# sp-uhh/audio-visual-vad

Measured on NVIDIA B200. Metric: AV-VAD frames/sec (device-timed), higher is better.
Workload: dtype bf16

## Files before the change

### audio-visual-vad_b200/csrc/lstm.cu

```cuda
#include <stdlib.h>

#include <mutex>
#include <string>

#include <vector>

#include "lstm_persist.cuh"
#include "lstm_pair.cuh"

namespace avvad {

__global__ void pack_lstm_w_kernel(const float* __restrict__ w, int H, int I, int ld, __nv_bfloat16* __restrict__ out) {
  const int64_t idx = (int64_t)blockIdx.x * blockDim.x + threadIdx.x;
  const int64_t total = (int64_t)4 * H * ld;
  if (idx >= total) return;
  const int np = (int)(idx / ld), j = (int)(idx - (int64_t)np * ld);
  const int u = np >> 2, g = np & 3;
  out[idx] = __float2bfloat16_rn(j < I ? w[(int64_t)(g * H + u) * I + j] : 0.f);
}
__global__ void pack_lstm_b_kernel(const float* __restrict__ b_ih, const float* __restrict__ b_hh, int H,
                                   float* __restrict__ out) {
  const int np = blockIdx.x * blockDim.x + threadIdx.x;
  if (np >= 4 * H) return;
  const int u = np >> 2, g = np & 3;
// ... 520 lines not shown
  static int n_chunks_pref = [] {
    const char* e = getenv("AVVAD_LSTM_CHUNKS");
    int v = e ? atoi(e) : 8;
    return v < 1 ? 1 : (v > 32 ? 32 : v);
  }();
  int n_chunks = n_chunks_pref;
  while (n_chunks > 1 && T / n_chunks < 16) --n_chunks;
  if (persistent && h->layers == 2 && n_chunks > 1) {
    int dev = 0;
    AVVAD_CUDA(cudaGetDevice(&dev));
    if (!h->side || h->side_device != dev) {
      if (h->side) cudaStreamDestroy(h->side);
      for (auto& e : h->ev_chunk) {
        if (e) cudaEventDestroy(e);
        e = nullptr;
      }
      if (h->ev_done) cudaEventDestroy(h->ev_done);
      h->ev_done = nullptr;
      AVVAD_CUDA(cudaStreamCreateWithFlags(&h->side, cudaStreamNonBlocking));
      for (auto& e : h->ev_chunk) AVVAD_CUDA(cudaEventCreateWithFlags(&e, cudaEventDisableTiming));
      AVVAD_CUDA(cudaEventCreateWithFlags(&h->ev_done, cudaEventDisableTiming));
      h->side_device = dev;
    }
    __nv_bfloat16* out0 = ws.hseq[0];
    __nv_bfloat16* out1 = ws.hseq[1];
    TapeView tv0{}, tv1{};
    if (tape) {
      tv0 = tape_layer(tape, 0, H, B, T);
      tv1 = tape_layer(tape, 1, H, B, T);
      out0 = tv0.hseq;
      out1 = tv1.hseq;
    }
    const int64_t Bp = (B + 127) / 128 * 128;
    int rc = tc::launch_tma_gemm_xt(layer_in, ld_in, h->w_ih[0], ld_in, B, T, T, H4, (int)ld_in, h->bias[0], ws.xproj, st);
    if (rc) return rc;
    const int free_sms = lstm_num_sms() - 2 * (4 * H / 128);
    for (int c = 0; c < n_chunks; ++c) {
      const int t0 = (int)(T * c / n_chunks), t1 = (int)(T * (c + 1) / n_chunks);
      bool done = false;
      rc = run_recurrence_persistent(h, 0, ws.xproj, out0, lengths, B, T, ws.counters, st, &done, tv0.gates, tv0.c, t0, t1,
                                     ws.c);
      if (rc) return rc;
      if (!done) {
        set_error("lstm: persistent recurrence unavailable");
        return AVVAD_ERR_STATE;
      }
      AVVAD_CUDA(cudaEventRecord(h->ev_chunk[c], st));
      AVVAD_CUDA(cudaStreamWaitEvent(h->side, h->ev_chunk[c], 0));
      rc = tc::launch_tma_gemm_xt(out0 + (int64_t)t0 * H, H, h->w_ih[1], H, B, t1 - t0, T, H4, H, h->bias[1],
                                  ws.xproj1 + (int64_t)t0 * H4 * Bp, h->side, free_sms > 16 ? free_sms : 0);
      if (rc) return rc;
      rc = run_recurrence_persistent(h, 1, ws.xproj1, out1, lengths, B, T, ws.counters + kCounterBytes / 4, h->side, &done,
                                     tv1.gates, tv1.c, t0, t1, ws.c1);
      if (rc) return rc;
    }
    AVVAD_CUDA(cudaEventRecord(h->ev_done, h->side));
    AVVAD_CUDA(cudaStreamWaitEvent(st, h->ev_done, 0));
    layer_out = out1;
  } else {
  for (int l = 0; l < h->layers; ++l) {
    layer_out = ws.hseq[l & 1];
    TapeView tv{};
    if (tape) {
      tv = tape_layer(tape, l, H, B, T);
      layer_out = tv.hseq;
    }
    int rc = persistent ? tc::launch_tma_gemm_xt(layer_in, ld_in, h->w_ih[l], ld_in, B, T, T, H4, (int)ld_in, h->bias[l],
                                                 ws.xproj, st)
                        : avvad_gemm_bf16(layer_in, ld_in, h->w_ih[l], ld_in, h->bias[l], ws.xproj, H4, 0, 0, rows, H4,
                                          ld_in, st);
    if (rc) return rc;
// ... 89 lines not shown
```

### audio-visual-vad_b200/csrc/lstm_pair.cuh

```cuda
#pragma once
#include "lstm_persist.cuh"

namespace avvad {
namespace tc {

__host__ __device__ constexpr int kPairThreadsOf(int epi_warps) { return 64 + 32 * epi_warps; }
__host__ __device__ constexpr int kPairStagesOf(int np) { return np == 128 ? 6 : 9; }
constexpr int kPairTraceSlots = 12;

struct PairGeom {
  int B, T, H, KB;
  int n_pairs;
  const float4* xT;
  int Bp;
  __nv_bfloat16* hseq;
  const int32_t* lengths;
  unsigned int* counters;
  __nv_bfloat16* gates_out;
  float* c_out;
  int t0, t1;
  float* c_state;
  unsigned long long* trace;
  int variant;
};
// ... 105 lines not shown
  const uint32_t tmem_acc = *tmem_slot;
  const uint32_t bar0_leader = mapa_u32(bar0, 0);
  auto LBAR = [&](int i) { return bar0_leader + 8u * (uint32_t)i; };

  if (warp == 0) {
    uint32_t it = 0;
    for (int t = (g.t0 > 1 ? g.t0 : 1); t < g.t1; ++t) {
      const unsigned int target = (unsigned int)(t - g.t0);
      bool ok = false;
      int kb = 0;
      uint32_t spins = 0;
      while (kb < g.KB) {
        if (!ok) {
          if (kPerKb == 2) {
            if (lane >= g.n_pairs) {
              ok = true;
            } else {
              unsigned int fv;
              asm volatile("ld.relaxed.gpu.global.u32 %0, [%1];" : "=r"(fv) : "l"(flags + lane) : "memory");
              ok = fv >= target;
            }
          } else {
            if (2 * lane >= g.n_pairs) {
              ok = true;
            } else {
              unsigned long long fv;
              asm volatile("ld.relaxed.gpu.global.u64 %0, [%1];" : "=l"(fv) : "l"(flags + 2 * lane) : "memory");
              ok = ((unsigned int)fv >= target) && ((unsigned int)(fv >> 32) >= target);
            }
          }
          if (++spins > (1u << 26)) __trap();
        }
        const unsigned int m = __ballot_sync(0xffffffffu, ok);
        if (lane == 0 && ((m >> (2 * kb)) & 3u) == 3u) {
          if (kTrace && kb == 0) trace[t * kPairTraceSlots + 0] = globaltimer_ns();
          if (g.variant & 2) asm volatile("fence.acq_rel.gpu;" ::: "memory");
          if (g.variant & 4) fence_proxy_async_global();
        }
        while (kb < g.KB && ((m >> (2 * kb)) & 3u) == 3u) {
          if (lane == 0) {
            const int s = it % S;
            mbar_wait(BAR(S + s), ((it / S) & 1u) ^ 1u);
            if (rank == 0) mbar_arrive_expect_tx(BAR(s), 32768u);
            tma_load_3d_2sm(sA + s * 16384u, &maps.h, kb * 64, t - 1, (int)rank * 128, LBAR(s));
            if (kTrace && kb == 0) trace[t * kPairTraceSlots + 1] = globaltimer_ns();
          }
          ++kb;
          ++it;
        }
      }
      if (kTrace && lane == 0) trace[t * kPairTraceSlots + 2] = globaltimer_ns();
    }
  } else if (warp == 1) {
    if (rank == 0) {
      constexpr uint32_t idesc = make_idesc_pair(NP);
      uint32_t it = 0;
      const int tb = g.t0 > 1 ? g.t0 : 1;
      for (int t = tb; t < g.t1; ++t) {
        const uint32_t k = (uint32_t)(t - tb), a = k & 1u;
        if (k >= 2) mbar_wait(BAR(kBarTE + a), ((k >> 1) - 1u) & 1u);
        tc_fence_after();
        const uint32_t d = tmem_acc + a * (uint32_t)NP;
        for (int kb = 0; kb < g.KB; ++kb, ++it) {
          const int s = it % S;
          mbar_wait(BAR(s), (it / S) & 1u);
          tc_fence_after();
          if (elect_one_sync()) {
            if (kTrace && kb == 0) trace[t * kPairTraceSlots + 3] = globaltimer_ns();
            const uint32_t a_lo = desc_lo(sA + s * 16384u);
            const uint32_t b_lo = desc_lo(sW + kb * kWTile);
// ... 87 lines not shown
            const float gg = tanh_hw(__uint_as_float(v[o + 2]) + x[u].z);
            const float go = sigmoid_hw(__uint_as_float(v[o + 3]) + x[u].w);
            c[u] = gf * c[u] + gi_ * gg;
            hv[j] = go * tanh_hw(c[u]);
            gp.v[2 * j] = pack_bf16x2(gi_, gf);
            gp.v[2 * j + 1] = pack_bf16x2(gg, go);
          }
          hp[4 * gi + 2 * k] = live ? pack_bf16x2(hv[0], hv[1]) : 0u;
          hp[4 * gi + 2 * k + 1] = live ? pack_bf16x2(hv[2], hv[3]) : 0u;
          if (gsave) st_global_256(gsave + 32 * gi + 16 * k, gp);
        }
      }
      if (row_ok) {
        if (kU == 16) {
          u32x8 o;
#pragma unroll
          for (int e = 0; e < 8; ++e) o.v[e] = hp[e & (kU / 2 - 1)];
          st_global_256(hrow + (int64_t)t * g.H, o);
        } else {
          *reinterpret_cast<uint4*>(hrow + (int64_t)t * g.H) = make_uint4(hp[0], hp[1], hp[2], hp[3]);
        }
        if (g.c_out) {
          float* cp = g.c_out + ((int64_t)b * g.T + t) * g.H + unit0;
#pragma unroll
          for (int k = 0; k < kU / 8; ++k) {
            u32x8 o;
#pragma unroll
            for (int e = 0; e < 8; ++e) o.v[e] = __float_as_uint(c[8 * k + e]);
            st_global_256(cp + 8 * k, o);
          }
        }
      }
      if (tr) trace[t * kPairTraceSlots + 7] = globaltimer_ns();
      asm volatile("bar.sync 1, %0;" ::"n"(32 * kEW) : "memory");
      if (warp == 2 && lane == 0) {
        if (kTrace) trace[t * kPairTraceSlots + 9] = globaltimer_ns();
        asm volatile("st.release.gpu.global.u32 [%0], %1;" ::"l"(flags + pair), "r"((unsigned int)(t + 1 - g.t0))
                     : "memory");
        if (kTrace) trace[t * kPairTraceSlots + 10] = globaltimer_ns();
      }
    }
    if (row_ok && g.c_state) {
      float4* cs = reinterpret_cast<float4*>(g.c_state + (int64_t)b * g.H + unit0);
#pragma unroll
      for (int u = 0; u < kU / 4; ++u) cs[u] = make_float4(c[4 * u], c[4 * u + 1], c[4 * u + 2], c[4 * u + 3]);
    }
  }

  tc_fence_before();
  __syncthreads();
  cluster_sync_all();
  if (warp == 1) {
    __syncwarp();
    tmem_dealloc2(tmem_acc, 2 * NP);
  }
}

}
}
```

### audio-visual-vad_b200/csrc/lstm_persist.cuh

```cuda
#pragma once
#include "gemm_tma.cuh"

namespace avvad {
namespace tc {

constexpr int kLstmThreads = 320;
constexpr int kLstmStages = 6;
constexpr int kLstmMaxSlices = 64;

struct LstmGeom {
  int B, T, H, KB;
  int n_slices;
  const float4* xT;
  int Bp;
  __nv_bfloat16* hseq;
  const int32_t* lengths;
  unsigned int* counters;
  __nv_bfloat16* gates_out;
  float* c_out;
  int t0, t1;
  float* c_state;
  int cluster;
  int variant;
};
// ... 118 lines not shown
              if (++spins > (1u << 26)) __trap();
            }
            if (elect_one_sync()) {
              asm volatile("fence.acq_rel.gpu;" ::: "memory");
              fence_proxy_async_global();
              tma_load_3d_mc(sA + s * 16384u, &maps.h, kb * 64, t - 1, ms * 128, BAR(s), cmask);
            }
            __syncwarp();
          }
        }
      }
    } else {
    const int f0 = 2 * lane, f1 = 2 * lane + 1;
    const unsigned long long* fpair = reinterpret_cast<const unsigned long long*>(flags + f0);
    for (int t = (g.t0 > 1 ? g.t0 : 1); t < g.t1; ++t) {
      const unsigned int target = (unsigned int)(t - g.t0);
      bool ok = false;
      int kb = 0;
      uint32_t spins = 0;
      while (kb < g.KB) {
        if (!ok) {
          if (f0 >= g.n_slices) {
            ok = true;
          } else {
            unsigned long long fv;
            asm volatile("ld.relaxed.gpu.global.u64 %0, [%1];" : "=l"(fv) : "l"(fpair) : "memory");
            ok = ((unsigned int)fv >= target) && (f1 >= g.n_slices || (unsigned int)(fv >> 32) >= target);
          }
          if (++spins > (1u << 26)) __trap();
          if (!ok && (g.variant & 2)) __nanosleep(20);
        }
        const unsigned int m = __ballot_sync(0xffffffffu, ok);
        if (lane == 0 && kb < g.KB && ((m >> (2 * kb)) & 3u) == 3u) {
          if (g.variant & 32) asm volatile("fence.acq_rel.gpu;" ::: "memory");
          if (g.variant & 64) fence_proxy_async_global();
        }
        while (kb < g.KB && ((m >> (2 * kb)) & 3u) == 3u) {
          if (lane == 0) {
            const int s = it % kLstmStages;
            mbar_wait(BAR(kLstmStages + s), ((it / kLstmStages) & 1u) ^ 1u);
            mbar_arrive_expect_tx(BAR(s), 16384u);
            tma_load_3d(sA + s * 16384u, &maps.h, kb * 64, t - 1, ms * 128, BAR(s));
          }
          ++kb;
          ++it;
        }
      }
    }
    }
  } else if (warp == 1) {
    constexpr uint32_t idesc = make_idesc(64);
    mbar_wait(BAR(kBarW), 0);
    tc_fence_after();
    uint32_t it = 0;
    const int tb = g.t0 > 1 ? g.t0 : 1;
    for (int t = tb; t < g.t1; ++t) {
      const uint32_t k = (uint32_t)(t - tb), acc = k & 1u;
      if (k >= 2) mbar_wait(BAR(kBarTE + acc), ((k >> 1) - 1u) & 1u);
      tc_fence_after();
      const uint32_t d = tmem_acc + acc * 64u;
      for (int kb = 0; kb < g.KB; ++kb, ++it) {
        const int s = it % kLstmStages;
        mbar_wait(BAR(s), (it / kLstmStages) & 1u);
        tc_fence_after();
        if (elect_one_sync()) {
          const uint32_t a_lo = desc_lo(sA + s * 16384u);
          const uint32_t b_lo = desc_lo(sW + kb * 8192u);
          umma_f16_lo(d, a_lo, b_lo, idesc, kb != 0);
// ... 127 lines not shown
```

### audio-visual-vad_b200/csrc/stem_s2d.cuh

```cuda
#pragma once
#include "gemm_tc.cuh"

namespace avvad {
namespace tc {

constexpr int kS2Builders = 256;
constexpr int kS2BuilderWarps = kS2Builders / 32;
constexpr int kS2EpiWarps = 8;
constexpr int kS2EpiThreads = kS2EpiWarps * 32;
constexpr int kS2ChPerWarp = 64 / (kS2EpiWarps / 4);
constexpr int kS2Passes = kS2ChPerWarp / 16;
constexpr int kS2Items = (67 * 37 + kS2Builders - 1) / kS2Builders;
constexpr int kS2Threads = kS2Builders + 32 + kS2EpiThreads;
constexpr int kS2FramesPerBatch = 2;
constexpr int kS2RowsPerFrame = 37;
constexpr int kS2Pitch = 160;
constexpr int kS2PlaneRows = 83;
constexpr uint32_t kS2PlaneBytes = kS2PlaneRows * kS2Pitch;
constexpr int kS2EdgeRows = 132;
constexpr uint32_t kS2EdgeChunkBytes = kS2EdgeRows * 16;
constexpr uint32_t kS2EdgePlaneBytes = 2 * kS2EdgeChunkBytes;
constexpr uint32_t kS2BufBytes = 2 * kS2PlaneBytes + 2 * kS2EdgePlaneBytes;
constexpr uint32_t kS2WStepBytes = 256 * 32;
constexpr uint32_t kS2WBytes = 8 * kS2WStepBytes;
constexpr uint32_t kS2OnesBytes = 128 * 32;
constexpr int kS2RingRows = 32;
constexpr uint32_t kS2RingRowBytes = 16 * 128;
constexpr uint32_t kS2RingBytes = kS2RingRows * kS2RingRowBytes;
constexpr uint32_t kS2EdgeHpBytes = 80 * 128;
constexpr uint32_t kS2OffW = 2 * kS2BufBytes;
constexpr uint32_t kS2OffOnes = kS2OffW + kS2WBytes;
constexpr uint32_t kS2OffRing = kS2OffOnes + kS2OnesBytes;
constexpr uint32_t kS2OffEdgeHp = kS2OffRing + kS2RingBytes;
constexpr uint32_t kS2OffLut = kS2OffEdgeHp + kS2EdgeHpBytes;
constexpr uint32_t kS2OffBias = kS2OffLut + 512;
constexpr uint32_t kS2OffBar = kS2OffBias + 256;
constexpr uint32_t kS2StageBytes = 288 * 16;
constexpr uint32_t kS2OffStage = kS2OffBar + 128;
constexpr uint32_t kS2Smem = 1024 + kS2OffStage + 2 * kS2StageBytes;
static_assert(kS2Smem <= 227 * 1024, "stem kernel: shared memory");

struct StemS2Params {
  const float* frames;
  const uint8_t* src;
  const int32_t* n_src;
  const int32_t* n_out;
  int f_max, t_max, num, den;
  float mean, denom;
  int standardise;
  int64_t n_frames;
  int64_t first;
  const __nv_bfloat16* w1b;
  int64_t src_bytes;
  const float* bias;
  __nv_bfloat16* out;
  double* stats;
};

__device__ __forceinline__ uint32_t desc_lo_ns(uint32_t saddr, uint32_t lbo_bytes) {
  return ((saddr & 0x3FFFFu) >> 4) | ((lbo_bytes >> 4) << 16);
}
__device__ __forceinline__ uint32_t desc_hi_ns(uint32_t sbo_bytes) { return (sbo_bytes >> 4) | (1u << 14); }

__device__ __forceinline__ void umma_f16_ns(uint32_t tmem_d, uint32_t a_lo, uint32_t a_hi, uint32_t b_lo, uint32_t b_hi,
                                            uint32_t idesc, uint32_t accum) {
  asm volatile(
      "{\n\t.reg .pred p;\n\t.reg .b64 da, db;\n\t"
      "mov.b64 da, {%1, %2};\n\t"
      "mov.b64 db, {%3, %4};\n\t"
      "setp.ne.b32 p, %6, 0;\n\t"
      "tcgen05.mma.cta_group::1.kind::f16 [%0], da, db, %5, p;\n\t}"
      ::"r"(tmem_d), "r"(a_lo), "r"(a_hi), "r"(b_lo), "r"(b_hi), "r"(idesc), "r"(accum)
      : "memory");
}

__device__ __forceinline__ int s2_src_index(int k, int n_src, int num, int den) {
  long long v = ((long long)den * (2LL * k + 1) - 1) / (2LL * num);
  return v < n_src - 1 ? (int)v : n_src - 1;
}

__device__ __forceinline__ void named_bar_sync(int id, int nthreads) {
  asm volatile("bar.sync %0, %1;" ::"r"(id), "r"(nthreads) : "memory");
}

__device__ __forceinline__ uint32_t bf16x2_max(uint32_t a, uint32_t b) {
  uint32_t r;
  asm("max.bf16x2 %0, %1, %2;" : "=r"(r) : "r"(a), "r"(b));
  return r;
}

template <int MODE, bool STATS = false>
__global__ void __launch_bounds__(kS2Threads, 1) stem_s2d_kernel(const StemS2Params p) {
  extern __shared__ uint8_t smem_raw[];
  const uint32_t raw = smem_u32(smem_raw);
  const uint32_t base = (raw + 1023u) & ~1023u;
  uint8_t* smem = smem_raw + (base - raw);
  float* bias_s = reinterpret_cast<float*>(smem + kS2OffBias);
  unsigned short* lut = reinterpret_cast<unsigned short*>(smem + kS2OffLut);
  const uint32_t bar0 = base + kS2OffBar;
  auto BAR = [&](int i) { return bar0 + 8u * (uint32_t)i; };
  volatile uint32_t* tmem_slot = reinterpret_cast<volatile uint32_t*>(smem + kS2OffBar + 96);

  const int tid = threadIdx.x;
  const int warp = tid >> 5, lane = tid & 31;
  const int64_t n_batches = (p.n_frames + kS2FramesPerBatch - 1) / kS2FramesPerBatch;

  for (uint32_t i = tid; i < (2 * kS2BufBytes) / 16; i += kS2Threads)
    reinterpret_cast<uint4*>(smem)[i] = make_uint4(0u, 0u, 0u, 0u);
  for (int idx = tid; idx < 7 * 256 * 16; idx += kS2Threads) {
    const int e = idx & 15, n = (idx >> 4) & 255, fr = idx >> 12;
    const int s = n >> 6, ch = n & 63;
    const int fs = e - 2 * s;
    __nv_bfloat16 v = __float2bfloat16_rn(0.f);
    if (fs >= 0 && fs < 7) v = p.w1b[ch * 64 + fr * 7 + fs];
    const uint32_t off = kS2OffW + (uint32_t)fr * kS2WStepBytes + (uint32_t)(n >> 3) * 256u + (uint32_t)(e >> 3) * 128u +
                         (uint32_t)(n & 7) * 16u + (uint32_t)(e & 7) * 2u;
    *reinterpret_cast<__nv_bfloat16*>(smem + off) = v;
  }
  for (int idx = tid; idx < 256 * 16; idx += kS2Threads) {
    const int e = idx & 15, n = idx >> 4;
    const float bv = p.bias ? p.bias[n & 63] : 0.f;
    const __nv_bfloat16 hi = __float2bfloat16_rn(bv);
    __nv_bfloat16 v = __float2bfloat16_rn(0.f);
    if (e == 0) v = hi;
    if (e == 1) v = __float2bfloat16_rn(bv - __bfloat162float(hi));
    const uint32_t off = kS2OffW + 7u * kS2WStepBytes + (uint32_t)(n >> 3) * 256u + (uint32_t)(e >> 3) * 128u +
                         (uint32_t)(n & 7) * 16u + (uint32_t)(e & 7) * 2u;
    *reinterpret_cast<__nv_bfloat16*>(smem + off) = v;
  }
  for (uint32_t i = tid; i < kS2OnesBytes / 4; i += kS2Threads)
    reinterpret_cast<uint32_t*>(smem + kS2OffOnes)[i] = 0x3F803F80u;
  if (tid < 64) bias_s[tid] = p.bias ? p.bias[tid] : 0.f;
  if (MODE == 1 && tid < 256) {
    float v = (float)tid;
    if (p.standardise) v = (v - p.mean) / p.denom;
    const __nv_bfloat16 h = __float2bfloat16_rn(v);
    lut[tid] = *reinterpret_cast<const unsigned short*>(&h);
  }
  if (tid == 0) {
    for (int i = 0; i < 2; ++i) {
      mbar_init(BAR(0 + i), kS2Builders);
      mbar_init(BAR(2 + i), 1);
      mbar_init(BAR(4 + i), 1);
      mbar_init(BAR(6 + i), kS2EpiWarps);
    }
    fence_barrier_init();
  }
  if (warp == kS2BuilderWarps) {
    tmem_alloc(smem_u32(const_cast<uint32_t*>(tmem_slot)), 512);
    tmem_relinquish();
  }
  fence_proxy_async();
  tc_fence_before();
  __syncthreads();
  tc_fence_after();
  const uint32_t tmem_acc = *tmem_slot;

  if (warp < kS2BuilderWarps) {
    uint32_t px[MODE == 0 ? kS2Items : 1];
    uint4 ck0 = make_uint4(0u, 0u, 0u, 0u), ck1 = ck0;
    bool live_next = false;
    uint32_t mis_next = 0;
    auto load_chunk = [&](const uint8_t* ptr) -> uint4 {
      if (ptr >= p.src && ptr + 16 <= p.src + p.src_bytes) return __ldg(reinterpret_cast<const uint4*>(ptr));
      uint32_t w[4] = {0u, 0u, 0u, 0u};
      for (int i = 0; i < 16; ++i)
        if (ptr + i >= p.src && ptr + i < p.src + p.src_bytes) w[i >> 2] |= (uint32_t)__ldg(ptr + i) << (8 * (i & 3));
      return make_uint4(w[0], w[1], w[2], w[3]);
    };
    auto fetch = [&](int64_t n) {
      if (MODE == 1) live_next = false;
      if (n >= p.n_frames) return;
      if (MODE == 0) {
        const float* f32 = p.frames + n * (67 * 67);
#pragma unroll
        for (int j = 0; j < kS2Items; ++j) {
          const int item = tid + j * kS2Builders;
          const int r = item / 37, q = item - r * 37;
// ... 95 lines not shown
      for (int t = -1; t < n_main; ++t, ++g) {
        const uint32_t acc = g & 1u;
        mbar_wait(BAR(6 + acc), ((g >> 1) & 1u) ^ 1u);
        tc_fence_after();
        if (elect_one_sync()) {
          const uint32_t d = tmem_acc + acc * 256u;
          umma_f16_ns(d, desc_lo_ns(base + kS2OffOnes, 128u), b_hi, desc_lo_ns(base + kS2OffW + 7u * kS2WStepBytes, 128u),
                      b_hi, idesc, 0);
#pragma unroll
          for (int fr = 0; fr < 7; ++fr) {
            const int a = fr >> 1, b = fr & 1;
            uint32_t a_lo, a_hi;
            if (t < 0) {
              a_lo = desc_lo_ns(bufa + 2 * kS2PlaneBytes + (uint32_t)b * kS2EdgePlaneBytes + (uint32_t)a * 16u,
                                kS2EdgeChunkBytes);
              a_hi = a_hi_edge;
            } else {
              a_lo = desc_lo_ns(bufa + (uint32_t)b * kS2PlaneBytes + (uint32_t)(16 * t + a) * kS2Pitch, 16u);
              a_hi = a_hi_main;
            }
            const uint32_t b_lo = desc_lo_ns(base + kS2OffW + (uint32_t)fr * kS2WStepBytes, 128u);
            umma_f16_ns(d, a_lo, a_hi, b_lo, b_hi, idesc, 1);
          }
          umma_commit(BAR(4 + acc));
          if (t == n_main - 1) umma_commit(BAR(2 + buf));
        }
        __syncwarp();
      }
    }
  } else {
    const int ew = warp - (kS2BuilderWarps + 1);
    const int q = warp & 3;
    const int half = ew >> 2;
    const int etid = tid - (kS2Builders + 32);
    const int L = q * 32 + lane;
    uint8_t* ring = smem + kS2OffRing;
    uint8_t* edge_hp = smem + kS2OffEdgeHp;
    uint32_t g = 0;
    if (STATS) {
      float sa[kS2ChPerWarp], sq[kS2ChPerWarp];
#pragma unroll
      for (int c = 0; c < kS2ChPerWarp; ++c) sa[c] = sq[c] = 0.f;
      for (int64_t bi = blockIdx.x; bi < n_batches; bi += gridDim.x) {
        const int nf = (int)((p.n_frames - bi * kS2FramesPerBatch) < kS2FramesPerBatch
                                 ? (p.n_frames - bi * kS2FramesPerBatch)
                                 : kS2FramesPerBatch);
        const int n_rows = nf * kS2RowsPerFrame;
        const int n_main = (n_rows + 15) / 16;
        for (int t = -1; t < n_main; ++t, ++g) {
          const uint32_t acc = g & 1u;
          mbar_wait(BAR(4 + acc), (g >> 1) & 1u);
          tc_fence_after();
          const uint32_t t_row = tmem_acc + acc * 256u + ((uint32_t)(q * 32) << 16);
          const int yy = (t < 0) ? L : 16 * t + (L >> 3);
          const int y = yy % kS2RowsPerFrame;
          const bool live = (yy < n_rows) && (y < 34) && (t >= 0 || L < 80);
          const int s_first = (t < 0) ? 2 : 0;
#pragma unroll 1
          for (int pass = 0; pass < kS2Passes; ++pass) {
            const int ch0 = half * kS2ChPerWarp + pass * 16;
#pragma unroll
            for (int sft = 0; sft < 4; ++sft) {
              uint32_t v[16];
              tmem_ld16(t_row + (uint32_t)sft * 64u + ch0, v);
              tmem_ld_wait();
              if (live && sft >= s_first) {
#pragma unroll
                for (int c = 0; c < 16; ++c) {
                  const float x = __uint_as_float(v[c]);
                  if (kS2Passes == 1 || pass == 0) {
                    sa[c] += x;
                    sq[c] = fmaf(x, x, sq[c]);
                  } else {
                    sa[(16 + c) % kS2ChPerWarp] += x;
                    sq[(16 + c) % kS2ChPerWarp] = fmaf(x, x, sq[(16 + c) % kS2ChPerWarp]);
                  }
                }
              }
            }
          }
          tc_fence_before();
          __syncwarp();
          if (lane == 0) mbar_arrive(BAR(6 + acc));
        }
      }
#pragma unroll
      for (int c = 0; c < kS2ChPerWarp; ++c) {
        float a = sa[c], b = sq[c];
#pragma unroll
        for (int o = 16; o > 0; o >>= 1) {
          a += __shfl_xor_sync(0xffffffffu, a, o);
          b += __shfl_xor_sync(0xffffffffu, b, o);
        }
        if (lane == 0) {
          atomicAdd(p.stats + half * kS2ChPerWarp + c, (double)a);
          atomicAdd(p.stats + 64 + half * kS2ChPerWarp + c, (double)b);
        }
      }
    } else
    for (int64_t bi = blockIdx.x; bi < n_batches; bi += gridDim.x) {
      const int nf = (int)((p.n_frames - bi * kS2FramesPerBatch) < kS2FramesPerBatch
                               ? (p.n_frames - bi * kS2FramesPerBatch)
                               : kS2FramesPerBatch);
      const int n_rows = nf * kS2RowsPerFrame;
      const int n_main = (n_rows + 15) / 16;
      for (int t = -1; t < n_main; ++t, ++g) {
        const uint32_t acc = g & 1u;
        mbar_wait(BAR(4 + acc), (g >> 1) & 1u);
        tc_fence_after();
        const uint32_t t_row = tmem_acc + acc * 256u + ((uint32_t)(q * 32) << 16);
        if (t < 0) {
#pragma unroll 1
          for (int pass = 0; pass < kS2Passes; ++pass) {
            const int ch0 = half * kS2ChPerWarp + pass * 16;
            uint32_t v1[16], v2[16], v3[16];
            tmem_ld16(t_row + 64u + ch0, v1);
            tmem_ld16(t_row + 128u + ch0, v2);
            tmem_ld16(t_row + 192u + ch0, v3);
            tmem_ld_wait();
            if (L < 80) {
              uint32_t o[8];
#pragma unroll
              for (int c = 0; c < 8; ++c) {
                const float x0 = fmaxf(fmaxf(__uint_as_float(v1[2 * c]), __uint_as_float(v2[2 * c])), __uint_as_float(v3[2 * c]));
                const float x1 = fmaxf(fmaxf(__uint_as_float(v1[2 * c + 1]), __uint_as_float(v2[2 * c + 1])),
                                       __uint_as_float(v3[2 * c + 1]));
                o[c] = pack_relu_bf16x2(x0, x1);
              }
              uint8_t* rowp = edge_hp + L * 128;
              const int k0 = ch0 >> 3;
              *reinterpret_cast<uint4*>(rowp + (((k0) ^ (L & 7)) << 4)) = make_uint4(o[0], o[1], o[2], o[3]);
              *reinterpret_cast<uint4*>(rowp + (((k0 + 1) ^ (L & 7)) << 4)) = make_uint4(o[4], o[5], o[6], o[7]);
            }
          }
          tc_fence_before();
          __syncwarp();
          if (lane == 0) mbar_arrive(BAR(6 + acc));
          named_bar_sync(1, kS2EpiThreads);
          continue;
        }
        const int yy = 16 * t + (L >> 3);
        const int i = L & 7;
        uint8_t* rrow = ring + (uint32_t)(yy & (kS2RingRows - 1)) * kS2RingRowBytes;
#pragma unroll 1
        for (int pass = 0; pass < kS2Passes; ++pass) {
          const int ch0 = half * kS2ChPerWarp + pass * 16;
          uint32_t v0[16], v1[16], v2[16], v3[16];
          tmem_ld16(t_row + ch0, v0);
          tmem_ld16(t_row + 64u + ch0, v1);
          tmem_ld16(t_row + 128u + ch0, v2);
          tmem_ld16(t_row + 192u + ch0, v3);
          tmem_ld_wait();
          uint32_t oa[8], ob[8];
#pragma unroll
          for (int c = 0; c < 16; c += 2) {
            float pa[2], pb[2];
#pragma unroll
            for (int h = 0; h < 2; ++h) {
              const float s0 = __uint_as_float(v0[c + h]), s1 = __uint_as_float(v1[c + h]);
              const float s2 = __uint_as_float(v2[c + h]), s3 = __uint_as_float(v3[c + h]);
              float left = __shfl_up_sync(0xffffffffu, s3, 1);
              left = (i == 0) ? s0 : left;
              pa[h] = fmaxf(fmaxf(left, s0), s1);
              pb[h] = fmaxf(fmaxf(s1, s2), s3);
            }
            oa[c >> 1] = pack_relu_bf16x2(pa[0], pa[1]);
            ob[c >> 1] = pack_relu_bf16x2(pb[0], pb[1]);
          }
          if (yy < n_rows) {
            const int k0 = ch0 >> 3;
            uint8_t* pxa = rrow + (2 * i) * 128;
            uint8_t* pxb = pxa + 128;
            *reinterpret_cast<uint4*>(pxa + (((k0) ^ i) << 4)) = make_uint4(oa[0], oa[1], oa[2], oa[3]);
            *reinterpret_cast<uint4*>(pxa + (((k0 + 1) ^ i) << 4)) = make_uint4(oa[4], oa[5], oa[6], oa[7]);
            *reinterpret_cast<uint4*>(pxb + (((k0) ^ i) << 4)) = make_uint4(ob[0], ob[1], ob[2], ob[3]);
            *reinterpret_cast<uint4*>(pxb + (((k0 + 1) ^ i) << 4)) = make_uint4(ob[4], ob[5], ob[6], ob[7]);
          }
        }
        tc_fence_before();
        __syncwarp();
        if (lane == 0) mbar_arrive(BAR(6 + acc));
        named_bar_sync(1, kS2EpiThreads);

        {
          const int ch = etid & 7, rr = (etid >> 3) & 7, pg = etid >> 6;
          int ys = 16 * t + 2 * rr;
          int fi = (ys >= kS2RowsPerFrame) ? 1 : 0;
          int y = ys - fi * kS2RowsPerFrame;
          if ((y & 1) == 0) {
            ++ys; ++y;
            if (y == kS2RowsPerFrame) { y = 0; ++fi; }
          }
          if ((y & 1) && y <= 33 && ys < n_rows && fi < nf) {
            const int ph = y >> 1;
            const uint8_t* r0 = ring + (uint32_t)(ys & (kS2RingRows - 1)) * kS2RingRowBytes;
            const uint8_t* r1 = ring + (uint32_t)((ys - 1) & (kS2RingRows - 1)) * kS2RingRowBytes;
            const uint8_t* r2 = ring + (uint32_t)((ys - 2) & (kS2RingRows - 1)) * kS2RingRowBytes;
            const bool top = (y >= 2);
            __nv_bfloat16* orow = p.out + ((bi * kS2FramesPerBatch + fi) * 17 + ph) * (17 * 64) + ch * 8;
#pragma unroll
            for (int pw = pg; pw < 17; pw += kS2EpiThreads / 64) {
              uint4 a, b, c;
              if (pw < 16) {
                const uint32_t off = (uint32_t)pw * 128u + (uint32_t)((ch ^ (pw >> 1)) << 4);
                a = *reinterpret_cast<const uint4*>(r0 + off);
                b = *reinterpret_cast<const uint4*>(r1 + off);
                c = top ? *reinterpret_cast<const uint4*>(r2 + off) : b;
              } else {
                a = *reinterpret_cast<const uint4*>(edge_hp + ys * 128 + ((ch ^ (ys & 7)) << 4));
                b = *reinterpret_cast<const uint4*>(edge_hp + (ys - 1) * 128 + ((ch ^ ((ys - 1) & 7)) << 4));
                c = top ? *reinterpret_cast<const uint4*>(edge_hp + (ys - 2) * 128 + ((ch ^ ((ys - 2) & 7)) << 4)) : b;
              }
              uint4 m;
              m.x = bf16x2_max(bf16x2_max(a.x, b.x), c.x);
              m.y = bf16x2_max(bf16x2_max(a.y, b.y), c.y);
              m.z = bf16x2_max(bf16x2_max(a.z, b.z), c.z);
              m.w = bf16x2_max(bf16x2_max(a.w, b.w), c.w);
              *reinterpret_cast<uint4*>(orow + pw * 64) = m;
            }
          }
        }
        named_bar_sync(1, kS2EpiThreads);
      }
    }
  }

  tc_fence_before();
  __syncthreads();
  if (warp == kS2BuilderWarps) {
    __syncwarp();
    tmem_dealloc(tmem_acc, 512);
  }
}

}
}
```

Before: 2.138 million.

## Chunk layer-0 input projection per chunk and make memory-ordering fences default

Measured after the change: 2.136 million, median of 6. Within noise of the previous version (-0.1%).

```diff
diff --git a/audio-visual-vad_b200/csrc/lstm.cu b/audio-visual-vad_b200/csrc/lstm.cu
--- a/audio-visual-vad_b200/csrc/lstm.cu
+++ b/audio-visual-vad_b200/csrc/lstm.cu
@@ -576,11 +576,13 @@
       out1 = tv1.hseq;
     }
     const int64_t Bp = (B + 127) / 128 * 128;
-    int rc = tc::launch_tma_gemm_xt(layer_in, ld_in, h->w_ih[0], ld_in, B, T, T, H4, (int)ld_in, h->bias[0], ws.xproj, st);
-    if (rc) return rc;
     const int free_sms = lstm_num_sms() - 2 * (4 * H / 128);
     for (int c = 0; c < n_chunks; ++c) {
       const int t0 = (int)(T * c / n_chunks), t1 = (int)(T * (c + 1) / n_chunks);
+      int rc = tc::launch_tma_gemm_xt(layer_in + (int64_t)t0 * ld_in, ld_in, h->w_ih[0], ld_in, B, t1 - t0, T, H4, (int)ld_in,
+                                      h->bias[0], ws.xproj + (int64_t)t0 * H4 * Bp, st,
+                                      (c > 0 && free_sms > 16) ? free_sms : 0);
+      if (rc) return rc;
       bool done = false;
       rc = run_recurrence_persistent(h, 0, ws.xproj, out0, lengths, B, T, ws.counters, st, &done, tv0.gates, tv0.c, t0, t1,
                                      ws.c);
diff --git a/audio-visual-vad_b200/csrc/lstm_pair.cuh b/audio-visual-vad_b200/csrc/lstm_pair.cuh
--- a/audio-visual-vad_b200/csrc/lstm_pair.cuh
+++ b/audio-visual-vad_b200/csrc/lstm_pair.cuh
@@ -161,10 +161,22 @@
           if (++spins > (1u << 26)) __trap();
         }
         const unsigned int m = __ballot_sync(0xffffffffu, ok);
-        if (lane == 0 && ((m >> (2 * kb)) & 3u) == 3u) {
-          if (kTrace && kb == 0) trace[t * kPairTraceSlots + 0] = globaltimer_ns();
-          if (g.variant & 2) asm volatile("fence.acq_rel.gpu;" ::: "memory");
-          if (g.variant & 4) fence_proxy_async_global();
+        if (((m >> (2 * kb)) & 3u) == 3u) {
+          if (kTrace && kb == 0 && lane == 0) trace[t * kPairTraceSlots + 0] = globaltimer_ns();
+          int kb_end = kb + 1;
+          while (kb_end < g.KB && ((m >> (2 * kb_end)) & 3u) == 3u) ++kb_end;
+          const int lkb = lane >> 1;
+          if (!(g.variant & 2) && lkb >= kb && lkb < kb_end && kPerKb * lane < 2 * g.n_pairs) {
+            if (kPerKb == 2) {
+              unsigned int fv;
+              asm volatile("ld.acquire.gpu.global.u32 %0, [%1];" : "=r"(fv) : "l"(flags + lane) : "memory");
+            } else {
+              unsigned long long fv;
+              asm volatile("ld.acquire.gpu.global.u64 %0, [%1];" : "=l"(fv) : "l"(flags + 2 * lane) : "memory");
+            }
+          }
+          __syncwarp();
+          if (lane == 0 && !(g.variant & 4)) fence_proxy_async_global();
         }
         while (kb < g.KB && ((m >> (2 * kb)) & 3u) == 3u) {
           if (lane == 0) {
@@ -318,6 +330,8 @@
         }
       }
       if (tr) trace[t * kPairTraceSlots + 7] = globaltimer_ns();
+      if (!(g.variant & 8)) fence_proxy_async_global();
+      if (tr) trace[t * kPairTraceSlots + 8] = globaltimer_ns();
       asm volatile("bar.sync 1, %0;" ::"n"(32 * kEW) : "memory");
       if (warp == 2 && lane == 0) {
         if (kTrace) trace[t * kPairTraceSlots + 9] = globaltimer_ns();
diff --git a/audio-visual-vad_b200/csrc/lstm_persist.cuh b/audio-visual-vad_b200/csrc/lstm_persist.cuh
--- a/audio-visual-vad_b200/csrc/lstm_persist.cuh
+++ b/audio-visual-vad_b200/csrc/lstm_persist.cuh
@@ -174,8 +174,8 @@
         }
         const unsigned int m = __ballot_sync(0xffffffffu, ok);
         if (lane == 0 && kb < g.KB && ((m >> (2 * kb)) & 3u) == 3u) {
-          if (g.variant & 32) asm volatile("fence.acq_rel.gpu;" ::: "memory");
-          if (g.variant & 64) fence_proxy_async_global();
+          if (!(g.variant & 32)) asm volatile("fence.acq_rel.gpu;" ::: "memory");
+          if (!(g.variant & 64)) fence_proxy_async_global();
         }
         while (kb < g.KB && ((m >> (2 * kb)) & 3u) == 3u) {
           if (lane == 0) {
```

## Replace shared-ring epilogue with register pooling and per-warp carry barriers

Applied to the files above, without the earlier changes.

Result: no change. 2.126 million before, 2.135 million after (median of 6 runs) (+0.4%).

```diff
diff --git a/audio-visual-vad_b200/csrc/stem_s2d.cuh b/audio-visual-vad_b200/csrc/stem_s2d.cuh
--- a/audio-visual-vad_b200/csrc/stem_s2d.cuh
+++ b/audio-visual-vad_b200/csrc/stem_s2d.cuh
@@ -12,10 +12,12 @@
 constexpr int kS2Passes = kS2ChPerWarp / 16;
 constexpr int kS2Items = (67 * 37 + kS2Builders - 1) / kS2Builders;
 constexpr int kS2Threads = kS2Builders + 32 + kS2EpiThreads;
-constexpr int kS2FramesPerBatch = 2;
+constexpr int kS2FramesPerBatch = 3;
 constexpr int kS2RowsPerFrame = 37;
+constexpr int kS2BatchRows = kS2FramesPerBatch * kS2RowsPerFrame;
+constexpr int kS2MainTiles = (kS2BatchRows + 15) / 16;
 constexpr int kS2Pitch = 160;
-constexpr int kS2PlaneRows = 83;
+constexpr int kS2PlaneRows = 16 * kS2MainTiles + 3;
 constexpr uint32_t kS2PlaneBytes = kS2PlaneRows * kS2Pitch;
 constexpr int kS2EdgeRows = 132;
 constexpr uint32_t kS2EdgeChunkBytes = kS2EdgeRows * 16;
@@ -24,19 +26,24 @@
 constexpr uint32_t kS2WStepBytes = 256 * 32;
 constexpr uint32_t kS2WBytes = 8 * kS2WStepBytes;
 constexpr uint32_t kS2OnesBytes = 128 * 32;
-constexpr int kS2RingRows = 32;
-constexpr uint32_t kS2RingRowBytes = 16 * 128;
-constexpr uint32_t kS2RingBytes = kS2RingRows * kS2RingRowBytes;
-constexpr uint32_t kS2EdgeHpBytes = 80 * 128;
+constexpr int kS2CarrySlots = 4;
+constexpr uint32_t kS2CarrySlotBytes = 2 * 32 * 16;
+constexpr uint32_t kS2CarryBytes = kS2EpiWarps * kS2CarrySlots * kS2CarrySlotBytes;
+constexpr uint32_t kS2EdgeHpBytes = 16 * ((kS2BatchRows + 15) / 16) * 128;
+constexpr int kS2NumBars = 8 + kS2EpiWarps * kS2CarrySlots;
 constexpr uint32_t kS2OffW = 2 * kS2BufBytes;
 constexpr uint32_t kS2OffOnes = kS2OffW + kS2WBytes;
-constexpr uint32_t kS2OffRing = kS2OffOnes + kS2OnesBytes;
-constexpr uint32_t kS2OffEdgeHp = kS2OffRing + kS2RingBytes;
+constexpr uint32_t kS2OffCarry = kS2OffOnes + kS2OnesBytes;
+constexpr uint32_t kS2OffEdgeHp = kS2OffCarry + kS2CarryBytes;
 constexpr uint32_t kS2OffLut = kS2OffEdgeHp + kS2EdgeHpBytes;
 constexpr uint32_t kS2OffBias = kS2OffLut + 512;
 constexpr uint32_t kS2OffBar = kS2OffBias + 256;
+constexpr uint32_t kS2OffTmemSlot = kS2OffBar + 8 * kS2NumBars;
 constexpr uint32_t kS2StageBytes = 288 * 16;
-constexpr uint32_t kS2OffStage = kS2OffBar + 128;
+constexpr uint32_t kS2OffStage = kS2OffBar + 512;
+static_assert(kS2OffTmemSlot + 4 <= kS2OffStage, "stem kernel: barrier area");
+static_assert(kS2BatchRows <= 128, "stem kernel: the edge tile holds one stream row per accumulator row");
+static_assert(kS2EpiWarps == 8 && kS2Passes == 2, "stem kernel: the epilogue is written for 8 warps x 32 channels");
 constexpr uint32_t kS2Smem = 1024 + kS2OffStage + 2 * kS2StageBytes;
 static_assert(kS2Smem <= 227 * 1024, "stem kernel: shared memory");
 
@@ -88,6 +95,20 @@
   asm("max.bf16x2 %0, %1, %2;" : "=r"(r) : "r"(a), "r"(b));
   return r;
 }
+__device__ __forceinline__ uint4 bf16x2_max4(uint4 a, uint4 b) {
+  return make_uint4(bf16x2_max(a.x, b.x), bf16x2_max(a.y, b.y), bf16x2_max(a.z, b.z), bf16x2_max(a.w, b.w));
+}
+
+__device__ __forceinline__ void tmem_ld_16x256b_x2(uint32_t taddr, uint32_t (&v)[8]) {
+  asm volatile("tcgen05.ld.sync.aligned.16x256b.x2.b32 {%0, %1, %2, %3, %4, %5, %6, %7}, [%8];"
+               : "=r"(v[0]), "=r"(v[1]), "=r"(v[2]), "=r"(v[3]), "=r"(v[4]), "=r"(v[5]), "=r"(v[6]), "=r"(v[7])
+               : "r"(taddr)
+               : "memory");
+}
+
+__host__ __device__ constexpr int s2_col_channel(int c) {
+  return (c & 32) + 8 * ((c >> 1) & 3) + 2 * ((c >> 3) & 3) + (c & 1);
+}
 
 template <int MODE, bool STATS = false>
 __global__ void __launch_bounds__(kS2Threads, 1) stem_s2d_kernel(const StemS2Params p) {
@@ -99,7 +120,7 @@
   unsigned short* lut = reinterpret_cast<unsigned short*>(smem + kS2OffLut);
   const uint32_t bar0 = base + kS2OffBar;
   auto BAR = [&](int i) { return bar0 + 8u * (uint32_t)i; };
-  volatile uint32_t* tmem_slot = reinterpret_cast<volatile uint32_t*>(smem + kS2OffBar + 96);
+  volatile uint32_t* tmem_slot = reinterpret_cast<volatile uint32_t*>(smem + kS2OffTmemSlot);
 
   const int tid = threadIdx.x;
   const int warp = tid >> 5, lane = tid & 31;
@@ -109,7 +130,7 @@
     reinterpret_cast<uint4*>(smem)[i] = make_uint4(0u, 0u, 0u, 0u);
   for (int idx = tid; idx < 7 * 256 * 16; idx += kS2Threads) {
     const int e = idx & 15, n = (idx >> 4) & 255, fr = idx >> 12;
-    const int s = n >> 6, ch = n & 63;
+    const int s = n >> 6, ch = s2_col_channel(n & 63);
     const int fs = e - 2 * s;
     __nv_bfloat16 v = __float2bfloat16_rn(0.f);
     if (fs >= 0 && fs < 7) v = p.w1b[ch * 64 + fr * 7 + fs];
@@ -119,7 +140,7 @@
   }
   for (int idx = tid; idx < 256 * 16; idx += kS2Threads) {
     const int e = idx & 15, n = idx >> 4;
-    const float bv = p.bias ? p.bias[n & 63] : 0.f;
+    const float bv = p.bias ? p.bias[s2_col_channel(n & 63)] : 0.f;
     const __nv_bfloat16 hi = __float2bfloat16_rn(bv);
     __nv_bfloat16 v = __float2bfloat16_rn(0.f);
     if (e == 0) v = hi;
@@ -144,6 +165,8 @@
       mbar_init(BAR(4 + i), 1);
       mbar_init(BAR(6 + i), kS2EpiWarps);
     }
+    for (int i = 0; i < kS2EpiWarps * kS2CarrySlots; ++i) mbar_init(BAR(8 + i), 1);
+
     fence_barrier_init();
   }
   if (warp == kS2BuilderWarps) {
@@ -305,9 +328,7 @@
     const int ew = warp - (kS2BuilderWarps + 1);
     const int q = warp & 3;
     const int half = ew >> 2;
-    const int etid = tid - (kS2Builders + 32);
     const int L = q * 32 + lane;
-    uint8_t* ring = smem + kS2OffRing;
     uint8_t* edge_hp = smem + kS2OffEdgeHp;
     uint32_t g = 0;
     if (STATS) {
@@ -327,7 +348,7 @@
           const uint32_t t_row = tmem_acc + acc * 256u + ((uint32_t)(q * 32) << 16);
           const int yy = (t < 0) ? L : 16 * t + (L >> 3);
           const int y = yy % kS2RowsPerFrame;
-          const bool live = (yy < n_rows) && (y < 34) && (t >= 0 || L < 80);
+          const bool live = (yy < n_rows) && (y < 34);
           const int s_first = (t < 0) ? 2 : 0;
 #pragma unroll 1
           for (int pass = 0; pass < kS2Passes; ++pass) {
@@ -366,134 +387,157 @@
           b += __shfl_xor_sync(0xffffffffu, b, o);
         }
         if (lane == 0) {
-          atomicAdd(p.stats + half * kS2ChPerWarp + c, (double)a);
-          atomicAdd(p.stats + 64 + half * kS2ChPerWarp + c, (double)b);
-        }
-      }
-    } else
-    for (int64_t bi = blockIdx.x; bi < n_batches; bi += gridDim.x) {
-      const int nf = (int)((p.n_frames - bi * kS2FramesPerBatch) < kS2FramesPerBatch
-                               ? (p.n_frames - bi * kS2FramesPerBatch)
-                               : kS2FramesPerBatch);
-      const int n_rows = nf * kS2RowsPerFrame;
-      const int n_main = (n_rows + 15) / 16;
-      for (int t = -1; t < n_main; ++t, ++g) {
-        const uint32_t acc = g & 1u;
-        mbar_wait(BAR(4 + acc), (g >> 1) & 1u);
-        tc_fence_after();
-        const uint32_t t_row = tmem_acc + acc * 256u + ((uint32_t)(q * 32) << 16);
-        if (t < 0) {
-#pragma unroll 1
-          for (int pass = 0; pass < kS2Passes; ++pass) {
-            const int ch0 = half * kS2ChPerWarp + pass * 16;
-            uint32_t v1[16], v2[16], v3[16];
-            tmem_ld16(t_row + 64u + ch0, v1);
-            tmem_ld16(t_row + 128u + ch0, v2);
-            tmem_ld16(t_row + 192u + ch0, v3);
-            tmem_ld_wait();
-            if (L < 80) {
-              uint32_t o[8];
-#pragma unroll
-              for (int c = 0; c < 8; ++c) {
-                const float x0 = fmaxf(fmaxf(__uint_as_float(v1[2 * c]), __uint_as_float(v2[2 * c])), __uint_as_float(v3[2 * c]));
-                const float x1 = fmaxf(fmaxf(__uint_as_float(v1[2 * c + 1]), __uint_as_float(v2[2 * c + 1])),
-                                       __uint_as_float(v3[2 * c + 1]));
-                o[c] = pack_relu_bf16x2(x0, x1);
+          const int ch = s2_col_channel(half * kS2ChPerWarp + c);
+          atomicAdd(p.stats + ch, (double)a);
+          atomicAdd(p.stats + 64 + ch, (double)b);
+        }
+      }
+    } else {
+      const int gi = lane >> 2, u = lane & 3;
+      const int qp = (q + 3) & 3;
+      const int chunk = half * 4 + u;
+      const int bar_out = 8 + (half * 4 + q) * kS2CarrySlots, bar_in = 8 + (half * 4 + qp) * kS2CarrySlots;
+      uint8_t* carry_out = smem + kS2OffCarry + (uint32_t)(half * 4 + q) * kS2CarrySlots * kS2CarrySlotBytes;
+      const uint8_t* carry_in = smem + kS2OffCarry + (uint32_t)(half * 4 + qp) * kS2CarrySlots * kS2CarrySlotBytes;
+      for (int64_t bi = blockIdx.x; bi < n_batches; bi += gridDim.x) {
+        const int nf = (int)((p.n_frames - bi * kS2FramesPerBatch) < kS2FramesPerBatch
+                                 ? (p.n_frames - bi * kS2FramesPerBatch)
+                                 : kS2FramesPerBatch);
+        const int n_rows = nf * kS2RowsPerFrame;
+        const int n_main = (n_rows + 15) / 16;
+        __nv_bfloat16* out_b = p.out + bi * kS2FramesPerBatch * (17 * 17 * 64) + chunk * 8;
+        auto out_px = [&](int r, int pw) {
+          const int fi = r / kS2RowsPerFrame, y = r - fi * kS2RowsPerFrame;
+          return reinterpret_cast<uint4*>(out_b + ((fi * 17 + (y >> 1)) * 17 + pw) * 64);
+        };
+        auto trigger = [&](int r) {
+          const int y = r % kS2RowsPerFrame;
+          return (y & 1) && y <= 33 && r < n_rows;
+        };
+        auto has_top = [&](int r) { return r % kS2RowsPerFrame >= 2; };
+        for (int t = -1; t < n_main; ++t, ++g) {
+          const uint32_t acc = g & 1u, slot = g % kS2CarrySlots;
+          mbar_wait(BAR(4 + acc), (g >> 1) & 1u);
+          tc_fence_after();
+          const uint32_t t_q = tmem_acc + acc * 256u + ((uint32_t)(q * 32) << 16) + (uint32_t)(half * 32);
+          if (t < 0) {
+            uint32_t e[4][4];
+#pragma unroll
+            for (int pass = 0; pass < 2; ++pass) {
+              uint32_t v[2][3][8];
+#pragma unroll
+              for (int h = 0; h < 2; ++h)
+#pragma unroll
+                for (int s = 1; s < 4; ++s)
+                  tmem_ld_16x256b_x2(t_q + ((uint32_t)(16 * h) << 16) + (uint32_t)(64 * s + 16 * pass), v[h][s - 1]);
+              tmem_ld_wait();
+#pragma unroll
+              for (int h = 0; h < 2; ++h)
+#pragma unroll
+                for (int m = 0; m < 2; ++m)
+#pragma unroll
+                  for (int k = 0; k < 2; ++k) {
+                    const int x = 4 * k + 2 * m;
+                    float o[2];
+#pragma unroll
+                    for (int c = 0; c < 2; ++c)
+                      o[c] = fmaxf(fmaxf(__uint_as_float(v[h][0][x + c]), __uint_as_float(v[h][1][x + c])),
+                                   __uint_as_float(v[h][2][x + c]));
+                    e[2 * h + m][2 * pass + k] = pack_relu_bf16x2(o[0], o[1]);
+                  }
+            }
+            tc_fence_before();
+            __syncwarp();
+            if (lane == 0) mbar_arrive(BAR(6 + acc));
+#pragma unroll
+            for (int j = 0; j < 4; ++j) {
+              const int r = 32 * q + 8 * j + gi;
+              if (r < n_rows)
+                *reinterpret_cast<uint4*>(edge_hp + r * 128 + ((chunk ^ gi) << 4)) =
+                    make_uint4(e[j][0], e[j][1], e[j][2], e[j][3]);
+            }
+            __syncwarp();
+            if (lane == 0) mbar_arrive(BAR(bar_out + slot));
+            if (q > 0) mbar_wait(BAR(bar_in + slot), (g / kS2CarrySlots) & 1u);
+#pragma unroll
+            for (int j = 0; j < 4; ++j) {
+              const int r = 32 * q + 8 * j + gi;
+              if (trigger(r)) {
+                auto row = [&](int rr) {
+                  return *reinterpret_cast<const uint4*>(edge_hp + rr * 128 + ((chunk ^ (rr & 7)) << 4));
+                };
+                uint4 mx = bf16x2_max4(make_uint4(e[j][0], e[j][1], e[j][2], e[j][3]), row(r - 1));
+                if (has_top(r)) mx = bf16x2_max4(mx, row(r - 2));
+                *out_px(r, 16) = mx;
               }
-              uint8_t* rowp = edge_hp + L * 128;
-              const int k0 = ch0 >> 3;
-              *reinterpret_cast<uint4*>(rowp + (((k0) ^ (L & 7)) << 4)) = make_uint4(o[0], o[1], o[2], o[3]);
-              *reinterpret_cast<uint4*>(rowp + (((k0 + 1) ^ (L & 7)) << 4)) = make_uint4(o[4], o[5], o[6], o[7]);
             }
+            continue;
+          }
+          uint32_t hp[4][2][4];
+#pragma unroll
+          for (int pass = 0; pass < 2; ++pass)
+#pragma unroll
+            for (int h = 0; h < 2; ++h) {
+              uint32_t v[4][8];
+#pragma unroll
+              for (int s = 0; s < 4; ++s)
+                tmem_ld_16x256b_x2(t_q + ((uint32_t)(16 * h) << 16) + (uint32_t)(64 * s + 16 * pass), v[s]);
+              tmem_ld_wait();
+#pragma unroll
+              for (int m = 0; m < 2; ++m)
+#pragma unroll
+                for (int k = 0; k < 2; ++k) {
+                  const int x = 4 * k + 2 * m;
+                  auto f = [&](int s, int c) { return __uint_as_float(v[s][x + c]); };
+                  const uint32_t left = __shfl_up_sync(0xffffffffu, pack_relu_bf16x2(f(3, 0), f(3, 1)), 4);
+                  const uint32_t p01 = pack_relu_bf16x2(fmaxf(f(0, 0), f(1, 0)), fmaxf(f(0, 1), f(1, 1)));
+                  hp[2 * h + m][0][2 * pass + k] = (gi == 0) ? p01 : bf16x2_max(left, p01);
+                  hp[2 * h + m][1][2 * pass + k] = pack_relu_bf16x2(fmaxf(fmaxf(f(1, 0), f(2, 0)), f(3, 0)),
+                                                                    fmaxf(fmaxf(f(1, 1), f(2, 1)), f(3, 1)));
+                }
           }
           tc_fence_before();
           __syncwarp();
           if (lane == 0) mbar_arrive(BAR(6 + acc));
-          named_bar_sync(1, kS2EpiThreads);
-          continue;
-        }
-        const int yy = 16 * t + (L >> 3);
-        const int i = L & 7;
-        uint8_t* rrow = ring + (uint32_t)(yy & (kS2RingRows - 1)) * kS2RingRowBytes;
-#pragma unroll 1
-        for (int pass = 0; pass < kS2Passes; ++pass) {
-          const int ch0 = half * kS2ChPerWarp + pass * 16;
-          uint32_t v0[16], v1[16], v2[16], v3[16];
-          tmem_ld16(t_row + ch0, v0);
-          tmem_ld16(t_row + 64u + ch0, v1);
-          tmem_ld16(t_row + 128u + ch0, v2);
-          tmem_ld16(t_row + 192u + ch0, v3);
-          tmem_ld_wait();
-          uint32_t oa[8], ob[8];
-#pragma unroll
-          for (int c = 0; c < 16; c += 2) {
-            float pa[2], pb[2];
-#pragma unroll
-            for (int h = 0; h < 2; ++h) {
-              const float s0 = __uint_as_float(v0[c + h]), s1 = __uint_as_float(v1[c + h]);
-              const float s2 = __uint_as_float(v2[c + h]), s3 = __uint_as_float(v3[c + h]);
-              float left = __shfl_up_sync(0xffffffffu, s3, 1);
-              left = (i == 0) ? s0 : left;
-              pa[h] = fmaxf(fmaxf(left, s0), s1);
-              pb[h] = fmaxf(fmaxf(s1, s2), s3);
+          auto row4 = [&](int j, int c) { return make_uint4(hp[j][c][0], hp[j][c][1], hp[j][c][2], hp[j][c][3]); };
+
+          const int r_first = 16 * t + 4 * q;
+          {
+            const int y0 = (r_first + 4) % kS2RowsPerFrame;
+            const bool two = (y0 & 1) && y0 >= 3;
+            uint4* cp = reinterpret_cast<uint4*>(carry_out + slot * kS2CarrySlotBytes);
+#pragma unroll
+            for (int c = 0; c < 2; ++c) cp[32 * c + lane] = two ? bf16x2_max4(row4(3, c), row4(2, c)) : row4(3, c);
+          }
+          __syncwarp();
+          if (lane == 0) mbar_arrive(BAR(bar_out + slot));
+
+          uint4 cin[2] = {};
+          if (trigger(r_first) || (trigger(r_first + 1) && has_top(r_first + 1))) {
+            const uint32_t gp = q ? g : g - 1;
+            mbar_wait(BAR(bar_in + gp % kS2CarrySlots), (gp / kS2CarrySlots) & 1u);
+            const uint4* cp = reinterpret_cast<const uint4*>(carry_in + (gp % kS2CarrySlots) * kS2CarrySlotBytes);
+#pragma unroll
+            for (int c = 0; c < 2; ++c) cin[c] = cp[32 * c + lane];
+          }
+#pragma unroll
+          for (int j = 0; j < 4; ++j) {
+            const int r = r_first + j;
+            if (!trigger(r)) continue;
+            const bool top = has_top(r);
+#pragma unroll
+            for (int c = 0; c < 2; ++c) {
+              uint4 mx;
+              if (j == 0) {
+                mx = bf16x2_max4(row4(0, c), cin[c]);
+              } else {
+                mx = bf16x2_max4(row4(j, c), row4(j - 1, c));
+                if (top) mx = bf16x2_max4(mx, j == 1 ? cin[c] : row4(j >= 2 ? j - 2 : 0, c));
+              }
+              *out_px(r, 2 * gi + c) = mx;
             }
-            oa[c >> 1] = pack_relu_bf16x2(pa[0], pa[1]);
-            ob[c >> 1] = pack_relu_bf16x2(pb[0], pb[1]);
-          }
-          if (yy < n_rows) {
-            const int k0 = ch0 >> 3;
-            uint8_t* pxa = rrow + (2 * i) * 128;
-            uint8_t* pxb = pxa + 128;
-            *reinterpret_cast<uint4*>(pxa + (((k0) ^ i) << 4)) = make_uint4(oa[0], oa[1], oa[2], oa[3]);
-            *reinterpret_cast<uint4*>(pxa + (((k0 + 1) ^ i) << 4)) = make_uint4(oa[4], oa[5], oa[6], oa[7]);
-            *reinterpret_cast<uint4*>(pxb + (((k0) ^ i) << 4)) = make_uint4(ob[0], ob[1], ob[2], ob[3]);
-            *reinterpret_cast<uint4*>(pxb + (((k0 + 1) ^ i) << 4)) = make_uint4(ob[4], ob[5], ob[6], ob[7]);
-          }
-        }
-        tc_fence_before();
-        __syncwarp();
-        if (lane == 0) mbar_arrive(BAR(6 + acc));
-        named_bar_sync(1, kS2EpiThreads);
-
-        {
-          const int ch = etid & 7, rr = (etid >> 3) & 7, pg = etid >> 6;
-          int ys = 16 * t + 2 * rr;
-          int fi = (ys >= kS2RowsPerFrame) ? 1 : 0;
-          int y = ys - fi * kS2RowsPerFrame;
-          if ((y & 1) == 0) {
-            ++ys; ++y;
-            if (y == kS2RowsPerFrame) { y = 0; ++fi; }
-          }
-          if ((y & 1) && y <= 33 && ys < n_rows && fi < nf) {
-            const int ph = y >> 1;
-            const uint8_t* r0 = ring + (uint32_t)(ys & (kS2RingRows - 1)) * kS2RingRowBytes;
-            const uint8_t* r1 = ring + (uint32_t)((ys - 1) & (kS2RingRows - 1)) * kS2RingRowBytes;
-            const uint8_t* r2 = ring + (uint32_t)((ys - 2) & (kS2RingRows - 1)) * kS2RingRowBytes;
-            const bool top = (y >= 2);
-            __nv_bfloat16* orow = p.out + ((bi * kS2FramesPerBatch + fi) * 17 + ph) * (17 * 64) + ch * 8;
-#pragma unroll
-            for (int pw = pg; pw < 17; pw += kS2EpiThreads / 64) {
-              uint4 a, b, c;
-              if (pw < 16) {
-                const uint32_t off = (uint32_t)pw * 128u + (uint32_t)((ch ^ (pw >> 1)) << 4);
-                a = *reinterpret_cast<const uint4*>(r0 + off);
-                b = *reinterpret_cast<const uint4*>(r1 + off);
-                c = top ? *reinterpret_cast<const uint4*>(r2 + off) : b;
-              } else {
-                a = *reinterpret_cast<const uint4*>(edge_hp + ys * 128 + ((ch ^ (ys & 7)) << 4));
-                b = *reinterpret_cast<const uint4*>(edge_hp + (ys - 1) * 128 + ((ch ^ ((ys - 1) & 7)) << 4));
-                c = top ? *reinterpret_cast<const uint4*>(edge_hp + (ys - 2) * 128 + ((ch ^ ((ys - 2) & 7)) << 4)) : b;
-              }
-              uint4 m;
-              m.x = bf16x2_max(bf16x2_max(a.x, b.x), c.x);
-              m.y = bf16x2_max(bf16x2_max(a.y, b.y), c.y);
-              m.z = bf16x2_max(bf16x2_max(a.z, b.z), c.z);
-              m.w = bf16x2_max(bf16x2_max(a.w, b.w), c.w);
-              *reinterpret_cast<uint4*>(orow + pw * 64) = m;
-            }
-          }
-        }
-        named_bar_sync(1, kS2EpiThreads);
+          }
+        }
       }
     }
   }
```
